# MarcVivas/gpu-physics-engine

Measured on AMD Instinct MI355X. Metric: physics_steps_per_sec, higher is better.
Workload: dtype f32+u32

## Files before the change

### gpu-physics-engine_amd/csrc/gpe_internal.h

```cpp
#pragma once

#include <hip/hip_runtime.h>
#include <stdint.h>

#include <string>
#include <vector>

#include "../../include/gpe.h"
#include "native_policy.h"

namespace gpe {

constexpr uint32_t kUnused = GPE_UNUSED_CELL_ID;
constexpr int kWave = 64;
constexpr int kStreamBlock = 256;
constexpr int kMaxStreamGrid = 256 * 8;

inline int stream_grid(uint64_t items, int per_block = kStreamBlock)
{
    uint64_t g = (items + per_block - 1) / per_block;
    if (g < 1) g = 1;
    if (g > (uint64_t)kMaxStreamGrid) g = kMaxStreamGrid;
    return (int)g;
}
// ... 243 lines not shown
constexpr int kNativeCtlSortsSeen = 38;
struct NativeState {
    NativePolicy policy;
    bool in_box = false;
    int32_t gx = 0, gy = 0;
    int passes = 4;
    uint32_t table_entries = 0;
    uint2 *block_table = nullptr;
    uint64_t table_cap = 0;
    uint32_t *keys = nullptr, *ids = nullptr;
    uint32_t *keys_b = nullptr, *ids_b = nullptr;
    uint64_t cap = 0;
    uint32_t *codes = nullptr;
    uint32_t *gkeys = nullptr, *gids = nullptr, *gkeys_b = nullptr, *gids_b = nullptr;
    uint64_t gcap = 0;
    uint2 *gtable = nullptr;
    uint32_t *ghist = nullptr;
    uint32_t ghist_set = 0;
    uint64_t gtable_cap = 0;
    const uint32_t *gsorted_ids_now = nullptr;
    uint32_t *exc_count = nullptr;
    uint2 *exc_entry = nullptr;
    uint64_t exc_tiles = 0, exc_cap = 0;
    uint4 *roster_hdr = nullptr;
    uint32_t *roster_ids = nullptr;
    uint64_t roster_cap = 0;
    TileBox tb;
    uint32_t *gho_count = nullptr;
    uint64_t gho_cap = 0;
    const uint32_t *gho_count_now = nullptr, *gho_entry_now = nullptr, *ghost_sort_now = nullptr;
    const uint32_t *exc_count_now = nullptr;
    const uint2 *exc_entry_now = nullptr;
    uint32_t *sorted_key = nullptr;
    bool sort_state_valid = false;
    uint64_t sorted_n = 0;
    uint32_t step_seq = 0;
    uint32_t collide_seq = 0;
    const uint32_t *fresh_word = nullptr;
    uint32_t reason = GPE_REASON_NO_PARTICLES;
    uint64_t native_steps = 0, compat_steps = 0;
    bool always_sort = false;
    int32_t blocks_x = 0, blocks_y = 0;
    int32_t bx0 = 0, by0 = 0;
    uint32_t *tile_ctl = nullptr;
    uint32_t *overflow1 = nullptr;
    uint64_t overflow_cap = 0;
    void *arena = nullptr;
    uint64_t arena_cap = 0;
    bool force = false;
    bool print_stats = false;
    uint32_t stat_calls = 0;
    uint32_t *host_stat = nullptr;
    uint32_t window_max = 0;
    unsigned long long *dbg_stamps = nullptr;
    uint4 *dbg_cycles = nullptr;
    uint64_t dbg_cycles_cap = 0;
};

constexpr int kShardMaxSlots = 9;
constexpr int kShardOwned = 0, kShardTotal = 1, kShardError = 2, kShardEpoch = 3, kShardHoles = 4;
constexpr int kShardSetWords = 8;
constexpr int kShardDoneTicket = 5;
struct ShardSlots {
    uint32_t n_slots;
    uint32_t rank[kShardMaxSlots];
    uint32_t send_off[kShardMaxSlots], send_cap_mig[kShardMaxSlots], send_cap_gho[kShardMaxSlots];
// ... 269 lines not shown
                            const uint32_t *ids, uint64_t n, float2 *pos_out, float2 *prev_out,
                            float *radius_out);
gpe_status launch_verlet(gpe_ctx *c, float2 *pos, float2 *prev, const float *radius, uint64_t n,
                         float dt);
gpe_status launch_build_cell_ids(gpe_ctx *c, const float2 *pos, const float *radius, uint64_t n,
                                 float cell_size, uint32_t *cell_ids, uint32_t *object_ids);
gpe_status sort_reserve(gpe_ctx *c, uint64_t n);
gpe_status sort_pairs(gpe_ctx *c, uint32_t *keys, uint32_t *vals, uint64_t n);
gpe_status sort_histogram(gpe_ctx *c, const uint32_t *keys, uint64_t n, uint32_t shift, uint32_t *hist256);
gpe_status sort_scatter_pass(gpe_ctx *c, const uint32_t *ka, const uint32_t *va, uint32_t *kb,
                             uint32_t *vb, uint64_t n, uint32_t shift);
gpe_status scan_reserve(gpe_ctx *c, uint64_t n);
gpe_status inclusive_scan(gpe_ctx *c, uint32_t *data, uint64_t n);
void sort_release(gpe_ctx *c);
void scan_release(gpe_ctx *c);
constexpr int kHistCopies = 8;
VerletParams verlet_params(const gpe_ctx *c, float dt);
gpe_status onesweep_reserve(gpe_ctx *c, uint64_t n);
void onesweep_release(gpe_ctx *c);
gpe_status onesweep_zero_hist(gpe_ctx *c);
struct OnesweepGate {
    const uint32_t *need = nullptr;
    uint32_t *key_copy = nullptr;
    uint32_t key_blocks_x = 1;
    uint64_t key_div_magic = 0;
    uint4 *table_reset = nullptr;
    uint64_t table_pairs = 0;
    uint32_t *fresh = nullptr;
    uint32_t *sorts = nullptr;
    uint32_t *sorts_seen = nullptr;
    int ticket_base = 0;
    const uint32_t *count_now = nullptr;
    uint32_t *sorted_count = nullptr;
};
gpe_status onesweep_sort(gpe_ctx *c, uint32_t *keys, uint32_t *vals, uint32_t *keys_b, uint32_t *vals_b,
                         uint64_t n, int passes, bool hist_ready, bool iota_vals, uint32_t **out_keys,
                         uint32_t **out_vals, bool bases_ready = false, uint2 *table = nullptr,
                         uint32_t table_entries = 0,
                         const uint32_t *hist_src = nullptr,
                         const OnesweepGate *gate = nullptr);
uint64_t remove_tiles(uint64_t n);
gpe_status launch_remove_count(gpe_ctx *c, const uint8_t *mask, float x, float y, float rr, uint32_t *tile_count,
                               unsigned long long *tile_key, unsigned long long *max_key);
gpe_status launch_remove_scatter(gpe_ctx *c, const uint8_t *mask, float x, float y, float rr,
                                 const uint32_t *tile_scanned, const uint32_t *uids = nullptr,
                                 uint32_t *uids_out = nullptr);
uint64_t query_tiles(uint64_t n);
gpe_status launch_query_count(gpe_ctx *c, bool box, const float *region, uint32_t *tile_count);
gpe_status launch_query_gather(gpe_ctx *c, bool box, const float *region, const uint32_t *tile_scanned,
                               uint32_t capacity, uint32_t *index_out, uint32_t *uid_out, float2 *pos_out,
                               float2 *prev_out, float *radius_out);
gpe_status launch_pick(gpe_ctx *c, float x, float y, unsigned long long *tile_key, unsigned long long *pick);
gpe_status native_configure(gpe_ctx *c);
bool native_should_run(gpe_ctx *c);
NativeStats native_read_stats(const NativeState &N);
void native_release(gpe_ctx *c);
gpe_status launch_shard_classify(gpe_ctx *c, const uint8_t *owner_of_block, const uint32_t *dest_mask_of_block,
                                 int32_t blocks_x, int32_t blocks_y, uint32_t my_rank, uint32_t *out_index,
                                 uint32_t *out_info, uint32_t *out_count, uint64_t out_capacity);
void shard_release(gpe_ctx *c);
void comm_release(gpe_ctx *c);
void ctl_release(gpe_ctx *c);
void shard_pack_args(gpe_ctx *c, PackArgs *P);
gpe_status coll_all_reduce_u32(gpe_ctx *c, uint32_t *d_buf, uint64_t count, uint32_t op);
gpe_status coll_all_to_all_u32(gpe_ctx *c, const uint32_t *d_send, const uint64_t *send_off, const uint64_t *send_cnt,
                               uint32_t *d_recv, const uint64_t *recv_off, const uint64_t *recv_cnt,
// ... 27 lines not shown
```

### gpu-physics-engine_amd/csrc/gpe_native.hip

```cpp
#include <assert.h>
#include <stdio.h>
#include <string.h>

#include <algorithm>
#include <string>
#include <utility>

#include "gpe_internal.h"
#include "native_launch.h"

namespace gpe {

template <class T>
static hipError_t release(gpe_ctx *c, T *&p)
{
    return dev_release(c, p);
}
template <class T>
static hipError_t reserve(gpe_ctx *c, T *&p, size_t payload, size_t slack, const char *tag)
{
    hipError_t e = release(c, p);
    if (e == hipSuccess) e = dev_reserve(c, &p, payload, slack, tag);
    return e;
}

void native_release(gpe_ctx *c)
{
    NativeState &N = c->native;
    void *bufs[] = {N.block_table, N.keys, N.ids, N.keys_b, N.ids_b, N.codes, N.sorted_key, N.gkeys, N.gids, N.gkeys_b,
                    N.gids_b, N.gtable, N.ghist, N.exc_count, N.gho_count, N.roster_hdr, N.roster_ids, N.tile_ctl,
                    N.overflow1, N.arena};
    for (void *b : bufs) (void)release(c, b);
    (void)release(c, N.dbg_stamps);
    (void)release(c, N.dbg_cycles);
    if (N.host_stat) (void)hipHostFree(N.host_stat);
    N = NativeState();
}

static gpe_status arena_reserve(gpe_ctx *c, uint64_t want);

NativeStats native_read_stats(const NativeState &N)
{
    assert(N.host_stat != nullptr);
    const auto word = [&](int k) { return __atomic_load_n(&N.host_stat[k], __ATOMIC_RELAXED); };
    NativeStats s;
    s.window_max = word(kStatWindowMax);
    s.arena = word(kStatArena);
    s.probe = word(kStatProbe);
    s.overflow = word(kStatOverflow);
    s.sub_tiles = word(kStatSubTiles);
    s.spills = word(kStatSpills);
    s.sorts = word(kStatSorts);
    s.overflow_new = word(kStatOverflowNew);
    s.halves_over = word(kStatHalvesOver);
    return s;
}

static void native_print_stats(gpe_ctx *c, const NativeStats &s)
{
    NativeState &N = c->native;
    if (N.print_stats && (++N.stat_calls & 127u) == 0)
        fprintf(stderr, "[gpe native] call %u: window max %u, arena slots used %u of %llu, 32x32 tiles over capacity %u, "
                        "quarters redone as 8x8 tiles %u, 8x8 tiles through the arena %u\n", N.stat_calls,
// ... 26 lines not shown
        for (int i = 0; i < 14; ++i) all += (double)h[i];
        for (int i = 0; i < 14; ++i)
            fprintf(stderr, "  P%d %.0f (%.1f%%)", i, h[16 + i] ? (double)h[i] / (double)h[16 + i] : 0.0, all > 0 ? 100.0 * (double)h[i] / all : 0.0);
        fprintf(stderr, "  (tiles %llu of %llu started)\n", h[16 + 6], h[16 + 0]);
        if (part == 1) (void)hipMemset(g_stamps, 0, 128 * 8);
    }
    return g_stamps;
}
#endif

static gpe_status native_prepare_step(gpe_ctx *c, uint32_t **sorted_ids, bool always_sort = false)
{
    NativeState &N = c->native;
    const uint64_t n = c->n;
    constexpr size_t kHistSet = (size_t)kHistCopies * 4 * 256;
    if (!c->os_ws.hist_clean) {
        GPE_HIP(c, hipMemsetAsync(c->os_ws.hist4, 0, 2 * kHistSet * sizeof(uint32_t), c->stream));
        c->os_ws.hist_clean = true;
        c->os_ws.hist_set = 0;
    }
    uint32_t *hist_now = c->os_ws.hist4 + (size_t)c->os_ws.hist_set * kHistSet;
    uint32_t *hist_next = c->os_ws.hist4 + (size_t)(c->os_ws.hist_set ^ 1u) * kHistSet;
    c->os_ws.hist_set ^= 1u;
    const uint32_t parity = (N.step_seq++) & 1u;
    const PreparePlan plan = N.policy.prepare(native_read_stats(N), always_sort, N.always_sort,
                                              (c->cfg.flags & GPE_FLAG_FUSED_HISTOGRAMS) != 0);
    const bool sharded = c->shard.on || c->use_order_keys || c->has_active_box;
    const bool kept_sharded = c->shard.on && c->shard.active && c->use_order_keys && N.gkeys != nullptr && !N.always_sort;
    const bool gated = N.passes >= 2 && (!sharded || kept_sharded);
    const bool reuse = gated && plan.keep_table && N.sort_state_valid && (kept_sharded || N.sorted_n == n) &&
                       N.exc_count != nullptr;
    const uint64_t pairs = ((uint64_t)N.table_entries + 1) / 2;
    const bool fuse_hist = plan.fuse_hist;
    HashGhosts hg;
    hg.sorted_count = N.tile_ctl + kCtlSortedCount;
    uint64_t g_bound = 0;
    if (kept_sharded) {
        const ShardState &SH = c->shard;
        g_bound = c->cap;
        const uint32_t epoch = __atomic_load_n(&SH.host_counts[kShardEpoch], __ATOMIC_ACQUIRE);
        if ((int32_t)(epoch - SH.begin_epoch) > 0) {
            const uint64_t gh = SH.host_counts[kShardTotal] >= SH.host_counts[kShardOwned]
                                    ? SH.host_counts[kShardTotal] - SH.host_counts[kShardOwned] : 0;
            g_bound = std::min<uint64_t>(c->cap, gh + std::max<uint64_t>(16384, gh / 4));
        }
        g_bound = std::min<uint64_t>(g_bound, n);
        hg.owned = SH.counts_now() + kShardOwned;
        hg.gkeys = N.gkeys; hg.gids = N.gids; hg.g_bound = g_bound;
        hg.gtable2 = (uint4 *)N.gtable; hg.gtable_pairs = pairs;
        hg.ghist_now = N.ghist + (size_t)N.ghist_set * kHistSet;
        hg.ghist_next = N.ghist + (size_t)(N.ghist_set ^ 1u) * kHistSet;
        N.ghist_set ^= 1u;
        hg.ghost_sort = N.tile_ctl + kCtlGhostSort + parity;
        hg.ghost_sort_next = N.tile_ctl + kCtlGhostSort + (parity ^ 1u);
        if (N.gho_count && N.gho_cap >= N.exc_tiles) {
            hg.gl_count = N.gho_count + (size_t)parity * N.exc_tiles;
            hg.gl_count_next = N.gho_count + (size_t)(parity ^ 1u) * N.exc_tiles;
            hg.gl_entry = N.gho_count + 2 * N.exc_tiles + (size_t)parity * N.exc_tiles * kGhostSlots;
        }
    }
    const uint64_t div_magic = ((1ull << 40) + (uint64_t)N.blocks_x - 1) / (uint64_t)N.blocks_x;
    {
        Scope s(c, "native/hash");
        const int grid = (int)std::min<uint64_t>(kHashGridMax, std::max<uint64_t>(1, n / (2ull * kHashBlock)));
        const uint32_t *n_valid = (c->shard.on && c->shard.active) ? c->shard.counts_now() + kShardTotal : nullptr;
        launch_native_hash(c, kept_sharded, grid, c->pos, c->radius, n, n_valid,
                           c->cell_size, N.gx, N.gy, N.bx0, N.by0, N.blocks_x, N.blocks_y, N.table_entries, N.keys,
                           N.codes, N.passes, hist_now, hist_next, c->os_ws.ctl, N.tile_ctl,
                           (uint4 *)N.block_table, gated ? 0ull : pairs,
                           N.host_stat, reuse ? N.sorted_key : nullptr, parity, div_magic,
                           N.exc_count ? N.exc_count + (size_t)parity * N.exc_tiles : nullptr,
                           N.exc_count ? N.exc_entry + (size_t)parity * N.exc_tiles * kExcSlots : nullptr,
                           N.exc_count ? N.exc_count + (size_t)(parity ^ 1u) * N.exc_tiles : nullptr, N.tb,
                           (uint32_t)std::max<uint64_t>(64, n >> 11),
                           fuse_hist ? 1u : 0u, hg);
        GPE_HIP(c, hipGetLastError());
    }
    uint32_t *sk = nullptr, *sv = nullptr;
    {
        Scope s(c, "native/sort");
        OnesweepGate g;
        g.need = N.tile_ctl + kCtlNeedSort + parity;
        if (reuse && !fuse_hist) {
            const int hgrid = (int)std::min<uint64_t>(kHistGatedGridMax, std::max<uint64_t>(1, n / (4ull * kHistGatedBlock)));
            launch_native_hist_gated(c, hgrid, N.keys, n, N.passes, hist_now, g.need);
            GPE_HIP(c, hipGetLastError());
        }
        g.fresh = N.tile_ctl + kCtlFresh + parity;
        g.sorts = N.tile_ctl + kCtlSorts;
        g.sorts_seen = N.tile_ctl + kCtlSortsSeen;
        if (gated) {
            g.key_copy = N.sorted_key; g.table_reset = (uint4 *)N.block_table; g.table_pairs = pairs;
            g.key_blocks_x = (uint32_t)N.blocks_x;
            g.key_div_magic = div_magic;
            g.count_now = hg.owned; g.sorted_count = N.tile_ctl + kCtlSortedCount;
        }
        GPE_TRY(onesweep_sort(c, N.keys, N.ids, N.keys_b, N.ids_b, n, N.passes, true, true, &sk, &sv, true,
                              N.block_table, N.table_entries, hist_now, &g));
    }
    (void)sk;
    N.gsorted_ids_now = nullptr;
    if (kept_sharded && g_bound > 0) {
        Scope s(c, "shard/ghost-sort");
        uint32_t *gk = nullptr, *gv = nullptr;
        OnesweepGate gg;
        gg.ticket_base = 8;
        gg.need = hg.ghost_sort;
        GPE_TRY(onesweep_sort(c, N.gkeys, N.gids, N.gkeys_b, N.gids_b, g_bound, N.passes, true, false, &gk, &gv, true,
                              N.gtable, N.table_entries, hg.ghist_now, &gg));
        (void)gk;
        N.gsorted_ids_now = gv;
    }
    N.sort_state_valid = gated;
    N.sorted_n = n;
    N.fresh_word = N.tile_ctl + kCtlFresh + parity;
    N.gho_count_now = hg.gl_count;
    N.gho_entry_now = hg.gl_entry;
    N.ghost_sort_now = hg.ghost_sort;
    N.exc_count_now = reuse ? N.exc_count + (size_t)parity * N.exc_tiles : nullptr;
    N.exc_entry_now = reuse ? N.exc_entry + (size_t)parity * N.exc_tiles * kExcSlots : nullptr;
    *sorted_ids = sv;
    return GPE_OK;
}
// ... 91 lines not shown
    if (!rosters_pay && N.roster_hdr) {
        N.roster_cap = 0;
        GPE_HIP(c, release(c, N.roster_hdr));
        GPE_HIP(c, release(c, N.roster_ids));
    }
    if (c->shard.on && c->has_active_box && N.gho_cap < N.exc_tiles) {
        N.gho_cap = 0;
        GPE_HIP(c, release(c, N.gho_count));
        if (reserve(c, N.gho_count, 2 * N.exc_tiles * (1 + (size_t)kGhostSlots) * sizeof(uint32_t), 64, "native.gho") == hipSuccess)
            N.gho_cap = N.exc_tiles;
    }
    if (N.gho_count) GPE_HIP(c, hipMemsetAsync(N.gho_count, 0, 2 * N.exc_tiles * sizeof(uint32_t), c->stream));
    if (rosters_pay && N.exc_count &&
        (c->cfg.flags & (GPE_FLAG_SORT_EVERY_STEP | GPE_FLAG_COUNTING_SORT_TILES)) == 0) {
        if (N.roster_cap < N.exc_tiles) {
            N.roster_cap = 0;
            GPE_HIP(c, release(c, N.roster_hdr));
            GPE_HIP(c, release(c, N.roster_ids));
            if (reserve(c, N.roster_hdr, N.exc_tiles * sizeof(uint4), 0, "native.roster_hdr") == hipSuccess &&
                reserve(c, N.roster_ids, N.exc_tiles * (size_t)kRosterCap * sizeof(uint32_t), 0, "native.roster_ids") == hipSuccess)
                N.roster_cap = N.exc_tiles;
            else { (void)release(c, N.roster_hdr); (void)release(c, N.roster_ids); }
        }
        if (N.roster_hdr) GPE_HIP(c, hipMemsetAsync(N.roster_hdr, 0, N.exc_tiles * sizeof(uint4), c->stream));
    }
    if (N.overflow_cap < tiles) {
        N.overflow_cap = 0;
        GPE_HIP(c, reserve(c, N.overflow1, (3 * tiles + 32 + 2 * kHintMax) * sizeof(uint32_t), 0, "native.overflow"));
        N.overflow_cap = tiles;
    }
    {
        const uint64_t want = std::min<uint64_t>(std::max<uint64_t>(c->cap, 1ull << 20), 32ull << 20);
        GPE_TRY(arena_reserve(c, std::max<uint64_t>(want, N.arena_cap)));
    }
    if (!N.tile_ctl) {
        GPE_HIP(c, reserve(c, N.tile_ctl, kCtlWords * sizeof(uint32_t), 0, "native.tile_ctl"));
        GPE_HIP(c, hipMemsetAsync(N.tile_ctl, 0, kCtlWords * sizeof(uint32_t), c->stream));
    }
    if (!N.host_stat) GPE_HIP(c, hipHostMalloc((void **)&N.host_stat, 64, hipHostMallocDefault));
    memset(N.host_stat, 0, 64);
    GPE_TRY(onesweep_reserve(c, c->cap));
    GPE_HIP(c, hipMemsetAsync(N.tile_ctl, 0, kCtlSorts * sizeof(uint32_t), c->stream));
    launch_native_check_box(c, c->pos, c->n,
                            (c->shard.on && c->shard.active) ? c->shard.counts_now() + kShardTotal : nullptr, c->cell_size, N.gx, N.gy,
                            N.tile_ctl + kCtlError);
    GPE_HIP(c, hipGetLastError());
    uint32_t flag = 1;
    GPE_HIP(c, hipMemcpyAsync(&flag, N.tile_ctl + kCtlError, sizeof(flag), hipMemcpyDeviceToHost, c->stream));
    GPE_HIP(c, hipStreamSynchronize(c->stream));
    GPE_HIP(c, hipMemsetAsync(N.tile_ctl, 0, kCtlSorts * sizeof(uint32_t), c->stream));
    N.reason = GPE_REASON_OUT_OF_BOX;
    if (flag != 0) return GPE_OK;
    N.in_box = true;
    const bool prof = c->profiling;
    c->profiling = false;
    uint32_t *ids = nullptr;
    gpe_status st = native_prepare_step(c, &ids, true);
    c->profiling = prof;
    GPE_TRY(st);
    launch_native_window_max(c, N.block_table, N.table_entries, N.blocks_x, N.blocks_y, N.tile_ctl + kCtlWindowMax);
    GPE_HIP(c, hipGetLastError());
    uint32_t wmax = 0xffffffffu;
    GPE_HIP(c, hipMemcpyAsync(&wmax, N.tile_ctl + kCtlWindowMax, sizeof(wmax), hipMemcpyDeviceToHost, c->stream));
    GPE_HIP(c, hipStreamSynchronize(c->stream));
    GPE_HIP(c, hipMemsetAsync(N.tile_ctl, 0, kCtlSorts * sizeof(uint32_t), c->stream));
    N.window_max = wmax;
// ... 236 lines not shown
```

### gpu-physics-engine_amd/csrc/k_native.hip

```cpp
#include <assert.h>
#include <stdio.h>
#include <stdlib.h>
#include <string.h>

#include <algorithm>
#include <type_traits>

#include "gpe_internal.h"
#include "k_pair.h"
#include "native_launch.h"

namespace gpe {

constexpr int kNatThreads = 512;
constexpr int kNatWaves = kNatThreads / 64;

__device__ __forceinline__ uint32_t nat_block_exclusive_scan(uint32_t v, uint32_t *s_w, uint32_t *total)
{
    const int lane = lane_id();
    const int w = (int)(threadIdx.x >> 6);
    const uint32_t inc = wave_inclusive_scan(v);
    if (lane == 63) s_w[w] = inc;
    __syncthreads();
    uint32_t base = 0, all = 0;
// ... 59 lines not shown
    }
    uint32_t over = 0;
    int k = 0;
#pragma unroll
    for (int y = -1; y <= 1; ++y) {
#pragma unroll
        for (int x = -1; x <= 1; ++x) {
            if (x == 0 && y == 0) continue;
            over |= (sx[x + 1] + sy[y + 1] < sq) ? (1u << k) : 0u;
            ++k;
        }
    }
    return over;
}

constexpr int kHashBatch = 2;
template <bool GHOSTS>
__global__ __launch_bounds__(kHashBlock, 8) void k_native_hash(const float2 *__restrict__ pos,
                                                            const float *__restrict__ radius, uint64_t n,
                                                            const uint32_t *__restrict__ n_valid_ptr,
                                                            float cell_size, int32_t gx, int32_t gy,
                                                            int32_t bx0, int32_t by0, int32_t blocks_x,
                                                            int32_t blocks_y, uint32_t pad_key,
                                                            uint32_t *__restrict__ keys,
                                                            uint32_t *__restrict__ codes, int digits,
                                                            uint32_t *hist4, uint32_t *__restrict__ hist_next,
                                                            uint32_t *__restrict__ os_ctl, uint32_t *tile_ctl,
                                                            uint4 *__restrict__ table2, uint64_t table_pairs,
                                                            uint32_t *__restrict__ host_stat,
                                                            const uint32_t *__restrict__ sorted_key, uint32_t parity,
                                                            uint64_t div_magic, uint32_t *__restrict__ exc_count,
                                                            uint2 *__restrict__ exc_entry,
                                                            uint32_t *__restrict__ exc_count_next, TileBox tb,
                                                            uint32_t straggler_limit, uint32_t fuse_always, HashGhosts G)
{
    (void)div_magic;
    __shared__ uint32_t s_hist[4 * 256];
    __shared__ uint32_t s_ghist[GHOSTS ? 4 * 256 : 1];
    __shared__ uint32_t s_sort_known;
    s_hist[threadIdx.x] = 0;
    if (GHOSTS) s_ghist[threadIdx.x] = 0;
    if (threadIdx.x == 0) s_sort_known = 0u;
    for (uint64_t i = (uint64_t)blockIdx.x * blockDim.x + threadIdx.x; i < table_pairs; i += (uint64_t)gridDim.x * blockDim.x)
        table2[i] = make_uint4(0xFFFFFFFFu, 0u, 0xFFFFFFFFu, 0u);
    if (GHOSTS)
    for (uint64_t i = (uint64_t)blockIdx.x * blockDim.x + threadIdx.x; i < G.gtable_pairs; i += (uint64_t)gridDim.x * blockDim.x)
        G.gtable2[i] = make_uint4(0xFFFFFFFFu, 0u, 0xFFFFFFFFu, 0u);
    if (exc_count_next) {
        const uint64_t nt = (uint64_t)tb.nx * (uint64_t)tb.ny;
        for (uint64_t i = (uint64_t)blockIdx.x * blockDim.x + threadIdx.x; i < nt; i += (uint64_t)gridDim.x * blockDim.x)
            exc_count_next[i] = 0;
    }
    if (GHOSTS && G.gl_count_next) {
        const uint64_t nt = (uint64_t)tb.nx * (uint64_t)tb.ny;
        for (uint64_t i = (uint64_t)blockIdx.x * blockDim.x + threadIdx.x; i < nt; i += (uint64_t)gridDim.x * blockDim.x)
            G.gl_count_next[i] = 0;
    }
    if (blockIdx.x == 0 && threadIdx.x < kCtlPerStepWords) {
        if (host_stat) {
            if (threadIdx.x == kCtlWindowMax) host_stat[kStatWindowMax] = tile_ctl[kCtlWindowMax];
            if (threadIdx.x == kCtlArena) host_stat[kStatArena] = tile_ctl[kCtlArena];
            if (threadIdx.x == kCtlOverflow1) {
                const uint32_t fresh_over = tile_ctl[kCtlOverflow1];
                host_stat[kStatOverflow] = fresh_over + tile_ctl[kCtlHintsSeen];
                host_stat[kStatOverflowNew] = fresh_over;
            }
            if (threadIdx.x == kCtlOverflow2) host_stat[kStatHalvesOver] = tile_ctl[kCtlOverflow2];
            if (threadIdx.x == kCtlSubTiles) host_stat[kStatSubTiles] = tile_ctl[kCtlSubTiles];
            if (threadIdx.x == kCtlSpills) host_stat[kStatSpills] = tile_ctl[kCtlSpills];
            if (threadIdx.x == 7) host_stat[kStatSorts] = tile_ctl[kCtlSorts];
        }
        tile_ctl[threadIdx.x] = 0;
    }
    if (blockIdx.x == 0) {
        for (int i = threadIdx.x; i < kHistCopies * 4 * 256; i += kHashBlock) hist_next[i] = 0;
        if (GHOSTS && G.ghist_next)
            for (int i = threadIdx.x; i < kHistCopies * 4 * 256; i += kHashBlock) G.ghist_next[i] = 0;
        if (threadIdx.x < 16) os_ctl[threadIdx.x] = 0;
        if (threadIdx.x == 0) {
            tile_ctl[kCtlNeedSort + (parity ^ 1u)] = 0;
            tile_ctl[kCtlFresh + (parity ^ 1u)] = 0;
            tile_ctl[parity ? kCtlStragglers0 : kCtlStragglers1] = 0;
            if (GHOSTS && G.ghost_sort_next) *G.ghost_sort_next = 0u;
            if (GHOSTS && G.gkeys && !G.gl_count) atomicOr(G.ghost_sort, 1u);
            if (!sorted_key) atomicOr(&tile_ctl[kCtlNeedSort + parity], 1u);
        }
    }
    __syncthreads();
    const uint64_t stride = (uint64_t)gridDim.x * blockDim.x;
    const uint64_t rounds = (n + stride - 1) / stride;
    uint64_t nv = n;
    if (n_valid_ptr) {
        nv = *n_valid_ptr;
        if (nv > n) { nv = n; if (threadIdx.x == 0) atomicOr(&tile_ctl[kCtlError], kErrBoundExceeded); }
    }
    uint64_t n_own = nv;
    if (GHOSTS && G.owned) n_own = min((uint64_t)*G.owned, nv);
    const uint64_t sorted_cnt = (sorted_key && G.sorted_count) ? (uint64_t)*G.sorted_count : ~0ull;
    if (GHOSTS && G.gkeys) {
        const uint64_t first = n - n_own;
        for (uint64_t j = first + (uint64_t)blockIdx.x * blockDim.x + threadIdx.x; j < G.g_bound; j += (uint64_t)gridDim.x * blockDim.x) {
            G.gkeys[j] = pad_key; G.gids[j] = 0u;
        }
        if (nv - n_own > G.g_bound && threadIdx.x == 0) atomicOr(&tile_ctl[kCtlError], kErrBoundExceeded);
    }
    bool oob = false, drifted = false;
    bool sort_known = sorted_key == nullptr;
    const bool fuse_hist = sorted_key == nullptr || fuse_always != 0u;
    for (uint64_t r0 = 0; r0 < rounds; r0 += kHashBatch) {
        float2 p[kHashBatch];
        float rad[kHashBatch];
        uint64_t idx[kHashBatch];
        uint32_t okey[kHashBatch];
#pragma unroll
        for (int u = 0; u < kHashBatch; ++u) {
            idx[u] = (r0 + u) * stride + (uint64_t)blockIdx.x * blockDim.x + threadIdx.x;
            const bool in = r0 + u < rounds && idx[u] < nv;
            p[u] = in ? pos[idx[u]] : make_float2(0.f, 0.f);
            rad[u] = in ? radius[idx[u]] : 0.f;
            okey[u] = (in && sorted_key) ? sorted_key[idx[u]] : 0u;
        }
#pragma unroll
        for (int u = 0; u < kHashBatch; ++u) {
            if (r0 + u >= rounds) break;
            const bool valid = idx[u] < n;
            uint32_t key = pad_key;
            if (valid && idx[u] >= nv) {
                keys[idx[u]] = pad_key; codes[idx[u]] = 0u;
                if (GHOSTS && G.gkeys && idx[u] - n_own < G.g_bound) { G.gkeys[idx[u] - n_own] = pad_key; G.gids[idx[u] - n_own] = 0u; }
            }
            const bool ghost = GHOSTS && idx[u] >= n_own;
            uint32_t gkey = 0;
            bool gvalid = false;
            if (idx[u] < nv) {
                const int32_t cx = cell_coord(p[u].x, cell_size), cy = cell_coord(p[u].y, cell_size);
                const int32_t lbx = (cx >> 3) - bx0, lby = (cy >> 3) - by0;
                const bool out = (cx < 0) | (cx >= gx) | (cy < 0) | (cy >= gy) | (lbx < 0) | (lbx >= blocks_x) |
                                 (lby < 0) | (lby >= blocks_y);
                oob |= out;
                key = out ? 0u : __umul24((uint32_t)lby, (uint32_t)blocks_x) + (uint32_t)lbx;
                if (GHOSTS && ghost && G.gkeys) {
// ... 15 lines not shown
                                (straggler ? kCodeStraggler : 0u);
                const uint64_t ms = ballot64(straggler);
                bool route = false;
                if (ms != 0 && !sort_known) {
                    sort_known = wave_lds_load(&s_sort_known) != 0u;
                    if (!sort_known) {
                        const int leader = (int)__builtin_ctzll(ms);
                        uint32_t before = 0;
                        if (lane_id() == leader)
                            before = atomicAdd(&tile_ctl[parity ? kCtlStragglers1 : kCtlStragglers0], (uint32_t)__popcll(ms));
                        before = (uint32_t)__builtin_amdgcn_readlane((int)before, leader);
                        if (before + (uint32_t)__popcll(ms) > straggler_limit) {
                            sort_known = true;
                            if (lane_id() == leader) { wave_lds_store(&s_sort_known, 1u); atomicOr(&tile_ctl[kCtlNeedSort + parity], 1u); }
                        } else route = true;
                    }
                }
                if (straggler && route) {
                    const int tx0 = max(tb.x0, (cx - (kConeRight + 1)) >> 5), tx1 = min(tb.x0 + tb.nx - 1, (cx + kConeLeft + 1) >> 5);
                    const int ty0 = max(tb.y0, (cy - (kConeUp + 1)) >> 5), ty1 = min(tb.y0 + tb.ny - 1, (cy + kConeDown + 1) >> 5);
                    for (int ty = ty0; ty <= ty1; ++ty)
                        for (int tx = tx0; tx <= tx1; ++tx) {
                            const uint32_t t = tb.index(tx, ty);
                            const uint32_t slot = atomicAdd(&exc_count[t], 1u);
                            if (slot < kExcSlots) exc_entry[(uint64_t)t * kExcSlots + slot] = make_uint2((uint32_t)idx[u], (uint32_t)cx | ((uint32_t)cy << 16));
                            else { drifted = true; atomicOr(&tile_ctl[kCtlNeedSort + parity], 1u); }
                        }
                }
            }
            if (fuse_hist) {
#pragma unroll
                for (int q = 0; q < 4; ++q)
                    if (q < digits) hist_add(s_hist + q * 256, (key >> (8 * q)) & 255u, valid);
            }
            if (GHOSTS && G.gkeys) {
#pragma unroll
                for (int q = 0; q < 4; ++q)
                    if (q < digits) hist_add(s_ghist + q * 256, (gkey >> (8 * q)) & 255u, gvalid);
            }
        }
    }
    if (GHOSTS && G.gl_count) {
        for (uint64_t i = n_own + (uint64_t)blockIdx.x * blockDim.x + threadIdx.x; i < nv; i += stride) {
            const float2 p = pos[i];
            const int32_t cx = cell_coord(p.x, cell_size), cy = cell_coord(p.y, cell_size);
            if ((cx < 0) | (cx >= gx) | (cy < 0) | (cy >= gy)) continue;
            const int tx0 = max(tb.x0, (cx - (kConeRight + 1)) >> 5), tx1 = min(tb.x0 + tb.nx - 1, (cx + kConeLeft + 1) >> 5);
            const int ty0 = max(tb.y0, (cy - (kConeUp + 1)) >> 5), ty1 = min(tb.y0 + tb.ny - 1, (cy + kConeDown + 1) >> 5);
            for (int ty = ty0; ty <= ty1; ++ty)
                for (int tx = tx0; tx <= tx1; ++tx) {
                    const uint32_t t = tb.index(tx, ty);
                    const uint32_t slot = atomicAdd(&G.gl_count[t], 1u);
                    if (slot < kGhostSlots) G.gl_entry[(uint64_t)t * kGhostSlots + slot] = (uint32_t)i;
                    else atomicOr(G.ghost_sort, 1u);
                }
        }
    }
    if (GHOSTS && G.gkeys && blockIdx.x == 0 && threadIdx.x < (uint32_t)digits) {
        const uint64_t ng = min(nv - n_own, G.g_bound);
        atomicAdd(&s_ghist[threadIdx.x * 256 + ((pad_key >> (8 * threadIdx.x)) & 255u)], (uint32_t)(G.g_bound - ng));
    }
    if (oob) atomicOr(&tile_ctl[kCtlError], kErrOutOfBox);
    if (ballot64(drifted) != 0 && lane_id() == 0) atomicOr(&tile_ctl[kCtlNeedSort + parity], 1u);
    __syncthreads();
    if ((threadIdx.x & 1u) == 0) {
        const uint32_t lo = s_hist[threadIdx.x], hi = s_hist[threadIdx.x + 1];
        if (fuse_hist && (lo | hi))
            __hip_atomic_fetch_add(
                reinterpret_cast<unsigned long long *>(&hist4[(blockIdx.x % kHistCopies) * 1024 + threadIdx.x]),
                (unsigned long long)lo | ((unsigned long long)hi << 32), __ATOMIC_RELAXED, __HIP_MEMORY_SCOPE_AGENT);
        if (GHOSTS && G.ghist_now) {
            const uint32_t glo = s_ghist[threadIdx.x], ghi = s_ghist[threadIdx.x + 1];
            if (glo | ghi)
                __hip_atomic_fetch_add(
                    reinterpret_cast<unsigned long long *>(&G.ghist_now[(blockIdx.x % kHistCopies) * 1024 + threadIdx.x]),
                    (unsigned long long)glo | ((unsigned long long)ghi << 32), __ATOMIC_RELAXED, __HIP_MEMORY_SCOPE_AGENT);
        }
    }
}

__global__ __launch_bounds__(kHistGatedBlock) void k_native_hist_gated(const uint32_t *__restrict__ keys, uint64_t n, int digits,
                                                                       uint32_t *__restrict__ hist4,
                                                                       const uint32_t *__restrict__ need)
{
    if (*need == 0u) return;
    __shared__ uint32_t s_hist[4 * 256];
    s_hist[threadIdx.x] = 0;
    __syncthreads();
    const uint64_t stride = (uint64_t)gridDim.x * blockDim.x;
    const uint64_t rounds = (n + stride - 1) / stride;
    for (uint64_t r = 0; r < rounds; ++r) {
        const uint64_t idx = r * stride + (uint64_t)blockIdx.x * blockDim.x + threadIdx.x;
        const bool valid = idx < n;
        const uint32_t key = valid ? keys[idx] : 0u;
#pragma unroll
        for (int q = 0; q < 4; ++q)
            if (q < digits) hist_add(s_hist + q * 256, (key >> (8 * q)) & 255u, valid);
// ... 2031 lines not shown
        A.tile_ctl[kCtlHintsSeen] = A.front_wgs != 0u ? used : 0u;
        A.tile_ctl[kCtlHints + A.hint_parity] = 0u;
    }
    if (work == 0) return;
    for (;;) {
        if (threadIdx.x == 0) s_item = atomicAdd(&A.tile_ctl[kCtlOverflowTicket], 1u);
        __syncthreads();
        const uint32_t i = s_item;
        __syncthreads();
        if (i >= work) break;
        uint32_t qx, qy;
        if (i >= work1) { const uint32_t h = A.overflow2[(i - work1) >> 1]; qx = (h & 0xFFFFu) * 2u + (i & 1u); qy = h >> 16; }
        else {
            const uint32_t parent = A.overflow1[i >> 2]; qx = (parent & 0xFFFFu) * 2u + (i & 1u); qy = (parent >> 16) * 2u + ((i >> 1) & 1u);
            if ((i & 3u) == 0u && threadIdx.x == 0) hint_tile(A, (int)(parent & 0xFFFFu), (int)(parent >> 16));
        }
#ifdef GPE_TILE_CYCLES
        const long long tq0 = clock64();
#endif
        resolve_quarter<ORD>(u, A, (int)qx, (int)qy);
#ifdef GPE_TILE_CYCLES
        if (g_tile_cycles && threadIdx.x == 0 && A.tb.holds((int)(qx >> 1), (int)(qy >> 1)))
            atomicAdd(&g_tile_cycles[A.tb.index((int)(qx >> 1), (int)(qy >> 1))].z, (uint32_t)(clock64() - tq0));
#endif
    }
}

void launch_native_hash(gpe_ctx *c, bool ghosts, int grid, const float2 *pos, const float *radius, uint64_t n,
                        const uint32_t *n_valid_ptr, float cell_size, int32_t gx, int32_t gy, int32_t bx0, int32_t by0,
                        int32_t blocks_x, int32_t blocks_y, uint32_t pad_key, uint32_t *keys, uint32_t *codes, int digits,
                        uint32_t *hist4, uint32_t *hist_next, uint32_t *os_ctl, uint32_t *tile_ctl, uint4 *table2,
                        uint64_t table_pairs, uint32_t *host_stat, const uint32_t *sorted_key, uint32_t parity,
                        uint64_t div_magic, uint32_t *exc_count, uint2 *exc_entry, uint32_t *exc_count_next, TileBox tb,
                        uint32_t straggler_limit, uint32_t fuse_always, const HashGhosts &G)
{
    const auto hash_kernel = ghosts ? k_native_hash<true> : k_native_hash<false>;
    hipLaunchKernelGGL(hash_kernel, dim3(grid), dim3(kHashBlock), 0, c->stream, pos, radius, n, n_valid_ptr, cell_size, gx,
                       gy, bx0, by0, blocks_x, blocks_y, pad_key, keys, codes, digits, hist4, hist_next, os_ctl, tile_ctl,
                       table2, table_pairs, host_stat, sorted_key, parity, div_magic, exc_count, exc_entry, exc_count_next,
                       tb, straggler_limit, fuse_always, G);
}

void launch_native_hist_gated(gpe_ctx *c, int grid, const uint32_t *keys, uint64_t n, int digits, uint32_t *hist4,
                              const uint32_t *need)
{
    hipLaunchKernelGGL(k_native_hist_gated, dim3(grid), dim3(kHistGatedBlock), 0, c->stream, keys, n, digits, hist4, need);
}

void launch_native_check_box(gpe_ctx *c, const float2 *pos, uint64_t n, const uint32_t *n_valid_ptr, float cell_size,
                             int32_t gx, int32_t gy, uint32_t *flag)
{
    hipLaunchKernelGGL(k_native_check_box, dim3(stream_grid(n)), dim3(kStreamBlock), 0, c->stream, pos, n, n_valid_ptr,
                       cell_size, gx, gy, flag);
}

void launch_native_window_max(gpe_ctx *c, const uint2 *table, uint32_t entries, int32_t blocks_x, int32_t blocks_y,
                              uint32_t *out_max)
{
    hipLaunchKernelGGL(k_native_window_max, dim3(stream_grid(entries)), dim3(kStreamBlock), 0, c->stream, table, entries,
                       blocks_x, blocks_y, out_max);
}

void launch_native_publish_probe(gpe_ctx *c, uint32_t *tile_ctl, uint32_t *host_stat)
{
    hipLaunchKernelGGL(k_native_publish_probe, dim3(1), dim3(64), 0, c->stream, tile_ctl, host_stat);
}

void launch_collide(gpe_ctx *c, CollideForm form, uint32_t grid, const CollideArgs &A)
{
    switch (form) {
    case CollideForm::DenseOrd:
        hipLaunchKernelGGL((k_collide_dense<kTileMain, kCapOrd, true>), dim3(grid), dim3(kNatThreads), 0, c->stream, A);
        break;
// ... 101 lines not shown
```

### gpu-physics-engine_amd/csrc/k_onesweep.hip

```cpp
#include <stdio.h>
#include <stdlib.h>

#include <algorithm>

#include "gpe_internal.h"

#ifdef GPE_OS_STAMPS
#define OS_STAMP(i)                                                                   \
    do {                                                                              \
        if (threadIdx.x == 0 && (s_tile & 63u) == 7u) {                               \
            const long long _t = clock64();                                           \
            atomicAdd(&ctl[16 + (i)], (uint32_t)(_t - _t_prev));                      \
            _t_prev = _t;                                                             \
        }                                                                             \
    } while (0)
#else
#define OS_STAMP(i) do {} while (0)
#endif

namespace gpe {

#ifndef GPE_OS_MINWAVES
#define GPE_OS_MINWAVES 4
#endif
// ... 117 lines not shown
    uint16_t slot[kOsItems];
#pragma unroll
    for (int k = 0; k < kOsItems; ++k) {
        const uint64_t idx = wave_base + (uint64_t)k * 64 + lane;
        const bool valid = idx < n;
        key[k] = valid ? keys_in[idx] : 0xffffffffu;
        if (IOTA) val[k] = (uint32_t)idx;
        else val[k] = valid ? vals_in[idx] : 0u;
    }
    if (G.key_copy) {
#pragma unroll
        for (int k = 0; k < kOsItems; ++k) {
            const uint64_t idx = wave_base + (uint64_t)k * 64 + lane;
            if (idx < n) {
                const uint32_t by = (uint32_t)(((uint64_t)key[k] * G.key_div_magic) >> 40);
                G.key_copy[idx] = (key[k] - by * G.key_blocks_x) | (by << 16);
            }
        }
        for (uint64_t i = (uint64_t)tile * kOsBlock + threadIdx.x; i < G.table_pairs; i += (uint64_t)gridDim.x * kOsBlock)
            G.table_reset[i] = make_uint4(0xFFFFFFFFu, 0u, 0xFFFFFFFFu, 0u);
        if (tile == 0 && threadIdx.x == 0) *G.sorted_count = G.count_now ? *G.count_now : (uint32_t)n;
    }
    if (G.fresh && tile == 0 && threadIdx.x == 0) {
        *G.fresh = 1u;
        const uint32_t before = atomicAdd(G.sorts, 1u);
        if (G.sorts_seen) *G.sorts_seen = before + 1u;
    }
    uint32_t digit_base = 0;
    if (hist_src) {
        uint32_t v = 0;
        if (threadIdx.x < 256) {
#pragma unroll
            for (int k = 0; k < kHistCopies; ++k) v += hist_src[k * 1024 + pass * 256 + threadIdx.x];
        }
        digit_base = os_block_exclusive_scan(v, s_w);
    }
#ifdef GPE_OS_STAMPS
    { uint32_t acc = 0; for (int k = 0; k < kOsItems; ++k) acc += key[k] + val[k]; asm volatile("" :: "v"(acc)); }
    OS_STAMP(0);
#endif
    uint32_t *wh = s_whist[w];
    u64 *wm = s_match[w];
    const u64 my_bit = 1ull << lane;
    constexpr int kBatch = 8;
    constexpr int kPeel = 4;
#pragma unroll
    for (int k0 = 0; k0 < kOsItems; k0 += kBatch) {
        u64 m[kBatch];
#pragma unroll
        for (int j = 0; j < kBatch; ++j) {
            const int k = k0 + j;
            const bool valid = wave_base + (uint64_t)k * 64 + lane < n;
            const uint32_t d = (key[k] >> shift) & 255u;
            u64 rem = ballot64(valid);
            u64 mine = 0ull;
#pragma unroll
            for (int it = 0; it < kPeel; ++it) {
                if (rem == 0) break;
                const int first = __builtin_amdgcn_readfirstlane((int)__builtin_ctzll(rem));
                const uint32_t d0 = (uint32_t)__builtin_amdgcn_readlane((int)d, first);
                const u64 same = ballot64(valid && d == d0) & rem;
                if (d == d0) mine = same;
                rem &= ~same;
            }
            const bool left = (rem >> lane) & 1ull;
            if (rem != 0) {
// ... 182 lines not shown
    if (passes < 1 || passes > 4) return fail(c, GPE_ERR_INVALID_ARG, "onesweep: passes must be 1..4");
    OnesweepWorkspace &ws = c->os_ws;
    const uint64_t tiles = os_tiles(n);
    if (!hist_ready) {
        Scope s(c, "sort/hist");
        GPE_TRY(onesweep_zero_hist(c));
        hipLaunchKernelGGL(k_os_hist4, dim3(stream_grid(n, kStreamBlock)), dim3(kStreamBlock), 0, c->stream, keys, n,
                           ws.hist_plain);
        GPE_HIP(c, hipGetLastError());
    }
    if (!(hist_ready && bases_ready)) {
        Scope s(c, "sort/prepare");
        hipLaunchKernelGGL(k_os_prepare, dim3(1), dim3(256), 0, c->stream, hist_ready ? ws.hist4 : ws.hist_plain, ws.bases4,
                           ws.ctl);
        GPE_HIP(c, hipGetLastError());
    }
    uint32_t *ka = keys, *va = vals, *kb = keys_b, *vb = vals_b;
    for (int p = 0; p < passes; ++p) {
        ws.epoch += 1;
        if (ws.epoch >= (1u << 30)) {
            GPE_HIP(c, hipMemsetAsync(ws.status, 0, ws.status_cap * sizeof(uint64_t), c->stream));
            ws.epoch = 1;
        }
        Scope s(c, "sort/onesweep");
        const bool iota = (p == 0 && iota_vals);
        const bool small = os_items(n) == kOsItemsSmall;
        const auto kern = small ? (iota ? k_os_pass<true, kOsItemsSmall> : k_os_pass<false, kOsItemsSmall>)
                                : (iota ? k_os_pass<true, kOsItems> : k_os_pass<false, kOsItems>);
        const bool last = p == passes - 1;
        OnesweepGate g;
        if (gate) {
            g.need = gate->need;
            g.ticket_base = gate->ticket_base;
            if (p == 0) {
                g.key_copy = gate->key_copy; g.table_reset = gate->table_reset; g.table_pairs = gate->table_pairs;
                g.key_blocks_x = gate->key_blocks_x; g.key_div_magic = gate->key_div_magic;
                g.count_now = gate->count_now; g.sorted_count = gate->sorted_count;
            }
            if (last) { g.fresh = gate->fresh; g.sorts = gate->sorts; g.sorts_seen = gate->sorts_seen; }
        }
        hipLaunchKernelGGL(kern, dim3((uint32_t)tiles), dim3(kOsBlock), 0, c->stream, ka, va, kb, vb, n,
                           (uint32_t)(8 * p), (uint32_t)p, ws.bases4, (u64 *)ws.status, ws.ctl, ws.epoch,
                           last ? table : nullptr, table_entries, (hist_ready && bases_ready) ? hist_src : nullptr, g);
        GPE_HIP(c, hipGetLastError());
        uint32_t *t = ka; ka = kb; kb = t;
        t = va; va = vb; vb = t;
    }
    if (out_keys) *out_keys = ka;
    if (out_vals) *out_vals = va;
#ifdef GPE_OS_STAMPS
    {
        static int calls = 0;
        if (++calls % 10 == 0) {
            uint32_t h[64];
            (void)hipStreamSynchronize(c->stream);
            (void)hipMemcpy(h, ws.ctl, sizeof(h), hipMemcpyDeviceToHost);
            const double nt = h[26] ? (double)h[26] : 1.0;
            fprintf(stderr, "[os stamps] n=%llu passes=%d sampled=%u  load %.0f  rank %.0f  reorder %.0f  lookback %.0f  write %.0f cyc;"
                            " hops/tile %.1f spins/tile %.1f\n", (unsigned long long)n, passes, h[26], h[16] / nt, h[17] / nt,
                    h[18] / nt, h[19] / nt, h[20] / nt, h[24] / nt, h[25] / nt);
        }
        (void)hipMemsetAsync(ws.ctl + 16, 0, 16 * sizeof(uint32_t), c->stream);
    }
#endif
    return GPE_OK;
}
// ... 3 lines not shown
```

### gpu-physics-engine_amd/csrc/native_launch.h

```cpp
#pragma once

#include "gpe_internal.h"

namespace gpe {

constexpr int kCtlOverflow1 = 0;
constexpr int kCtlOverflow2 = 1;
constexpr int kCtlHalfTicket = 7;
constexpr int kCtlWindowMax = 2;
constexpr int kCtlArena = 3;
constexpr int kCtlOverflowTicket = 4;
constexpr int kCtlSubTiles = 5;
constexpr int kCtlSpills = 6;
constexpr int kCtlPerStepWords = 8;
constexpr int kCtlHints = 11;
constexpr int kCtlHintsSeen = 13;
constexpr int kCtlError = 8;
constexpr int kCtlNeedSort = 34;
constexpr int kCtlFresh = 36;
constexpr int kCtlSorts = kNativeCtlSorts;
constexpr int kCtlStragglers0 = 9, kCtlStragglers1 = 15;
constexpr int kCtlSortedCount = 32;
constexpr int kCtlSortsSeen = kNativeCtlSortsSeen;
constexpr int kCtlGhostSort = 40;
constexpr int kCtlWords = 64;
constexpr uint32_t kExcSlots = 16;
constexpr uint32_t kGhostSlots = 256;
constexpr uint64_t kArenaBytesPerSlot = 37;
constexpr int kTileMain = 32;
struct HashGhosts {
    const uint32_t *owned = nullptr;
    uint32_t *gkeys = nullptr, *gids = nullptr;
    uint64_t g_bound = 0;
    uint4 *gtable2 = nullptr;
    uint64_t gtable_pairs = 0;
    const uint32_t *sorted_count = nullptr;
    uint32_t *ghist_now = nullptr, *ghist_next = nullptr;
    uint32_t *gl_count = nullptr, *gl_entry = nullptr, *gl_count_next = nullptr;
    uint32_t *ghost_sort = nullptr, *ghost_sort_next = nullptr;
};
constexpr int kHashBlock = 1024;
constexpr int kHashGridMax = 2048;
constexpr int kHistGatedBlock = 1024, kHistGatedGridMax = 2048;
#ifndef GPE_QMAX_MAIN_VALUE
#define GPE_QMAX_MAIN_VALUE 3
#endif
struct CollideArgs {
    const float2 *pos_in;
    const float *radius;
    float2 *pos_out;
    const uint32_t *sorted_ids;
    const uint32_t *codes;
    const uint2 *gtable;
    const uint32_t *gsorted_ids;
    const uint32_t *exc_count;
    const uint2 *exc_entry;
    TileBox tb;
    const uint32_t *gho_count;
    const uint32_t *gho_entry;
    const uint32_t *ghost_sort;
    const uint32_t *fresh;
    const uint2 *table;
    uint32_t entries;
    int32_t blocks_x, blocks_y;
    int32_t bx0, by0;
    const uint32_t *counts;
    float cell_size;
    float stiffness;
    int32_t gx, gy;
    int32_t tiles_x, tiles_y;
    uint32_t band_tiles;
    int32_t frame_l, frame_r, frame_b, frame_t;
    int32_t tile_x0, tile_y0;
    const uint32_t *order_keys;
    uint32_t *tile_ctl;
    uint32_t *overflow1;
    uint32_t overflow1_cap;
    uint32_t *overflow2;
    uint32_t quarters_of_halves;
    uint32_t *hints;
    uint32_t step_stamp, front_wgs, hint_parity;
    uint32_t hints_on;
    float *arena_px, *arena_py, *arena_rad;
    uint32_t *arena_id, *arena_hm, *arena_mem;
    uint8_t *arena_sblk;
    uint32_t arena_cap;
    float2 *prev;
    uint64_t n_owned;
    uint32_t fuse_verlet;
    VerletParams vp;
    uint4 *roster_hdr;
    uint32_t *roster_ids;
    const uint32_t *sorts_seen;
    uint32_t roster_write;
    unsigned long long *stamps;
    PackArgs pack;
};
constexpr int kRosterCap = GPE_QMAX_MAIN_VALUE * 512;

void launch_native_hash(gpe_ctx *c, bool ghosts, int grid, const float2 *pos, const float *radius, uint64_t n,
                        const uint32_t *n_valid_ptr, float cell_size, int32_t gx, int32_t gy, int32_t bx0, int32_t by0,
                        int32_t blocks_x, int32_t blocks_y, uint32_t pad_key, uint32_t *keys, uint32_t *codes, int digits,
                        uint32_t *hist4, uint32_t *hist_next, uint32_t *os_ctl, uint32_t *tile_ctl, uint4 *table2,
                        uint64_t table_pairs, uint32_t *host_stat, const uint32_t *sorted_key, uint32_t parity,
                        uint64_t div_magic, uint32_t *exc_count, uint2 *exc_entry, uint32_t *exc_count_next, TileBox tb,
                        uint32_t straggler_limit, uint32_t fuse_always, const HashGhosts &G);
void launch_native_hist_gated(gpe_ctx *c, int grid, const uint32_t *keys, uint64_t n, int digits, uint32_t *hist4,
                              const uint32_t *need);
void launch_native_check_box(gpe_ctx *c, const float2 *pos, uint64_t n, const uint32_t *n_valid_ptr, float cell_size,
                             int32_t gx, int32_t gy, uint32_t *flag);
void launch_native_window_max(gpe_ctx *c, const uint2 *table, uint32_t entries, int32_t blocks_x, int32_t blocks_y,
                              uint32_t *out_max);
void launch_native_publish_probe(gpe_ctx *c, uint32_t *tile_ctl, uint32_t *host_stat);
enum class CollideForm {
    Dense, DenseOrd,
    Direct, DirectFront, DirectOrd, DirectOrdFront,
    BorderOrd,
    Halves, HalvesOrd,
    Overflow, OverflowOrd,
};
void launch_collide(gpe_ctx *c, CollideForm form, uint32_t grid, const CollideArgs &A);
uint32_t dense_launch_band(uint32_t tiles_x, uint32_t tiles_y, bool eighths);
uint32_t dense_launch_grid(uint32_t tiles_x, uint32_t tiles_y, uint32_t band_tiles);

}
```

Baseline: 13390.

## Maintain radix histograms incrementally from key deltas instead of gated recount

When the sort table is reused and the run is not sharded, the hash kernel now adds only per-digit histogram deltas for particles whose cell key changed, rather than launching a separate gated histogram kernel over all keys. The onesweep sort adds a persistent kept histogram, stored in a double-buffered slot selected by a control word, to these deltas and writes the result back for the next step. This removes a full pass over the keys each step, at the cost of wave-level ballots and shared atomics in the hash kernel. It also adds cross-step state that must stay consistent with the actual sorted keys.

```diff
diff --git a/gpu-physics-engine_amd/csrc/gpe_internal.h b/gpu-physics-engine_amd/csrc/gpe_internal.h
--- a/gpu-physics-engine_amd/csrc/gpe_internal.h
+++ b/gpu-physics-engine_amd/csrc/gpe_internal.h
@@ -299,6 +299,7 @@
     const uint32_t *exc_count_now = nullptr;
     const uint2 *exc_entry_now = nullptr;
     uint32_t *sorted_key = nullptr;
+    uint32_t *kept_hist = nullptr;
     bool sort_state_valid = false;
     uint64_t sorted_n = 0;
     uint32_t step_seq = 0;
@@ -634,6 +635,9 @@
     int ticket_base = 0;
     const uint32_t *count_now = nullptr;
     uint32_t *sorted_count = nullptr;
+    uint32_t *kept = nullptr;
+    const uint32_t *kept_set = nullptr;
+    uint32_t kept_add = 0;
 };
 gpe_status onesweep_sort(gpe_ctx *c, uint32_t *keys, uint32_t *vals, uint32_t *keys_b, uint32_t *vals_b,
                          uint64_t n, int passes, bool hist_ready, bool iota_vals, uint32_t **out_keys,
diff --git a/gpu-physics-engine_amd/csrc/gpe_native.hip b/gpu-physics-engine_amd/csrc/gpe_native.hip
--- a/gpu-physics-engine_amd/csrc/gpe_native.hip
+++ b/gpu-physics-engine_amd/csrc/gpe_native.hip
@@ -28,7 +28,7 @@
 {
     NativeState &N = c->native;
     void *bufs[] = {N.block_table, N.keys, N.ids, N.keys_b, N.ids_b, N.codes, N.sorted_key, N.gkeys, N.gids, N.gkeys_b,
-                    N.gids_b, N.gtable, N.ghist, N.exc_count, N.gho_count, N.roster_hdr, N.roster_ids, N.tile_ctl,
+                    N.gids_b, N.gtable, N.ghist, N.kept_hist, N.exc_count, N.gho_count, N.roster_hdr, N.roster_ids, N.tile_ctl,
                     N.overflow1, N.arena};
     for (void *b : bufs) (void)release(c, b);
     (void)release(c, N.dbg_stamps);
@@ -121,6 +121,7 @@
                        N.exc_count != nullptr;
     const uint64_t pairs = ((uint64_t)N.table_entries + 1) / 2;
     const bool fuse_hist = plan.fuse_hist;
+    const bool delta_hist = reuse && !fuse_hist && !sharded && n <= kHistDeltaMaxN;
     HashGhosts hg;
     hg.sorted_count = N.tile_ctl + kCtlSortedCount;
     uint64_t g_bound = 0;
@@ -162,7 +163,7 @@
                            N.exc_count ? N.exc_entry + (size_t)parity * N.exc_tiles * kExcSlots : nullptr,
                            N.exc_count ? N.exc_count + (size_t)(parity ^ 1u) * N.exc_tiles : nullptr, N.tb,
                            (uint32_t)std::max<uint64_t>(64, n >> 11),
-                           fuse_hist ? 1u : 0u, hg);
+                           fuse_hist ? kHashHistFused : delta_hist ? kHashHistDelta : kHashHistGated, hg);
         GPE_HIP(c, hipGetLastError());
     }
     uint32_t *sk = nullptr, *sv = nullptr;
@@ -170,7 +171,7 @@
         Scope s(c, "native/sort");
         OnesweepGate g;
         g.need = N.tile_ctl + kCtlNeedSort + parity;
-        if (reuse && !fuse_hist) {
+        if (reuse && !fuse_hist && !delta_hist) {
             const int hgrid = (int)std::min<uint64_t>(kHistGatedGridMax, std::max<uint64_t>(1, n / (4ull * kHistGatedBlock)));
             launch_native_hist_gated(c, hgrid, N.keys, n, N.passes, hist_now, g.need);
             GPE_HIP(c, hipGetLastError());
@@ -178,6 +179,7 @@
         g.fresh = N.tile_ctl + kCtlFresh + parity;
         g.sorts = N.tile_ctl + kCtlSorts;
         g.sorts_seen = N.tile_ctl + kCtlSortsSeen;
+        g.kept = N.kept_hist; g.kept_set = N.tile_ctl + kCtlKeptSet; g.kept_add = delta_hist ? 1u : 0u;
         if (gated) {
             g.key_copy = N.sorted_key; g.table_reset = (uint4 *)N.block_table; g.table_pairs = pairs;
             g.key_blocks_x = (uint32_t)N.blocks_x;
@@ -335,6 +337,10 @@
     {
         const uint64_t want = std::min<uint64_t>(std::max<uint64_t>(c->cap, 1ull << 20), 32ull << 20);
         GPE_TRY(arena_reserve(c, std::max<uint64_t>(want, N.arena_cap)));
+    }
+    if (!N.kept_hist) {
+        GPE_HIP(c, reserve(c, N.kept_hist, 2 * 4 * 256 * sizeof(uint32_t), 0, "native.kept_hist"));
+        GPE_HIP(c, hipMemsetAsync(N.kept_hist, 0, 2 * 4 * 256 * sizeof(uint32_t), c->stream));
     }
     if (!N.tile_ctl) {
         GPE_HIP(c, reserve(c, N.tile_ctl, kCtlWords * sizeof(uint32_t), 0, "native.tile_ctl"));
diff --git a/gpu-physics-engine_amd/csrc/k_native.hip b/gpu-physics-engine_amd/csrc/k_native.hip
--- a/gpu-physics-engine_amd/csrc/k_native.hip
+++ b/gpu-physics-engine_amd/csrc/k_native.hip
@@ -115,7 +115,7 @@
                                                             uint64_t div_magic, uint32_t *__restrict__ exc_count,
                                                             uint2 *__restrict__ exc_entry,
                                                             uint32_t *__restrict__ exc_count_next, TileBox tb,
-                                                            uint32_t straggler_limit, uint32_t fuse_always, HashGhosts G)
+                                                            uint32_t straggler_limit, uint32_t hist_mode, HashGhosts G)
 {
     (void)div_magic;
     __shared__ uint32_t s_hist[4 * 256];
@@ -166,6 +166,7 @@
             tile_ctl[parity ? kCtlStragglers0 : kCtlStragglers1] = 0;
             if (GHOSTS && G.ghost_sort_next) *G.ghost_sort_next = 0u;
             if (GHOSTS && G.gkeys && !G.gl_count) atomicOr(G.ghost_sort, 1u);
+            tile_ctl[kCtlKeptSet] = tile_ctl[kCtlSorts] & 1u;
             if (!sorted_key) atomicOr(&tile_ctl[kCtlNeedSort + parity], 1u);
         }
     }
@@ -189,7 +190,8 @@
     }
     bool oob = false, drifted = false;
     bool sort_known = sorted_key == nullptr;
-    const bool fuse_hist = sorted_key == nullptr || fuse_always != 0u;
+    const bool fuse_hist = sorted_key == nullptr || hist_mode == kHashHistFused;
+    const bool delta_hist = !fuse_hist && hist_mode == kHashHistDelta;
     for (uint64_t r0 = 0; r0 < rounds; r0 += kHashBatch) {
         float2 p[kHashBatch];
         float rad[kHashBatch];
@@ -271,6 +273,19 @@
 #pragma unroll
                 for (int q = 0; q < 4; ++q)
                     if (q < digits) hist_add(s_hist + q * 256, (key >> (8 * q)) & 255u, valid);
+            } else if (delta_hist) {
+                const uint32_t old = __umul24(okey[u] >> 16, (uint32_t)blocks_x) + (okey[u] & 0xFFFFu);
+                const bool moved = valid && key != old;
+                if (ballot64(moved) != 0) {
+#pragma unroll
+                    for (int q = 0; q < 4; ++q) {
+                        const uint32_t d_new = (key >> (8 * q)) & 255u, d_old = (old >> (8 * q)) & 255u;
+                        if (q < digits && moved && d_new != d_old) {
+                            atomicAdd(&s_hist[q * 256 + d_new], 1u);
+                            atomicAdd(&s_hist[q * 256 + d_old], 0xFFFFFFFFu);
+                        }
+                    }
+                }
             }
             if (GHOSTS && G.gkeys) {
 #pragma unroll
@@ -302,6 +317,12 @@
     if (oob) atomicOr(&tile_ctl[kCtlError], kErrOutOfBox);
     if (ballot64(drifted) != 0 && lane_id() == 0) atomicOr(&tile_ctl[kCtlNeedSort + parity], 1u);
     __syncthreads();
+    if (delta_hist) {
+        const uint32_t v = s_hist[threadIdx.x];
+        if (v)
+            __hip_atomic_fetch_add(&hist4[(blockIdx.x % kHistCopies) * 1024 + threadIdx.x], v, __ATOMIC_RELAXED,
+                                   __HIP_MEMORY_SCOPE_AGENT);
+    }
     if ((threadIdx.x & 1u) == 0) {
         const uint32_t lo = s_hist[threadIdx.x], hi = s_hist[threadIdx.x + 1];
         if (fuse_hist && (lo | hi))
@@ -2399,13 +2420,13 @@
                         uint32_t *hist4, uint32_t *hist_next, uint32_t *os_ctl, uint32_t *tile_ctl, uint4 *table2,
                         uint64_t table_pairs, uint32_t *host_stat, const uint32_t *sorted_key, uint32_t parity,
                         uint64_t div_magic, uint32_t *exc_count, uint2 *exc_entry, uint32_t *exc_count_next, TileBox tb,
-                        uint32_t straggler_limit, uint32_t fuse_always, const HashGhosts &G)
+                        uint32_t straggler_limit, uint32_t hist_mode, const HashGhosts &G)
 {
     const auto hash_kernel = ghosts ? k_native_hash<true> : k_native_hash<false>;
     hipLaunchKernelGGL(hash_kernel, dim3(grid), dim3(kHashBlock), 0, c->stream, pos, radius, n, n_valid_ptr, cell_size, gx,
                        gy, bx0, by0, blocks_x, blocks_y, pad_key, keys, codes, digits, hist4, hist_next, os_ctl, tile_ctl,
                        table2, table_pairs, host_stat, sorted_key, parity, div_magic, exc_count, exc_entry, exc_count_next,
-                       tb, straggler_limit, fuse_always, G);
+                       tb, straggler_limit, hist_mode, G);
 }
 
 void launch_native_hist_gated(gpe_ctx *c, int grid, const uint32_t *keys, uint64_t n, int digits, uint32_t *hist4,
diff --git a/gpu-physics-engine_amd/csrc/k_onesweep.hip b/gpu-physics-engine_amd/csrc/k_onesweep.hip
--- a/gpu-physics-engine_amd/csrc/k_onesweep.hip
+++ b/gpu-physics-engine_amd/csrc/k_onesweep.hip
@@ -173,6 +173,11 @@
         if (threadIdx.x < 256) {
 #pragma unroll
             for (int k = 0; k < kHistCopies; ++k) v += hist_src[k * 1024 + pass * 256 + threadIdx.x];
+            if (G.kept) {
+                const uint32_t set = *G.kept_set & 1u;
+                if (G.kept_add) v += G.kept[set * 1024 + pass * 256 + threadIdx.x];
+                if (tile == 0) G.kept[(set ^ 1u) * 1024 + pass * 256 + threadIdx.x] = v;
+            }
         }
         digit_base = os_block_exclusive_scan(v, s_w);
     }
@@ -421,6 +426,7 @@
         if (gate) {
             g.need = gate->need;
             g.ticket_base = gate->ticket_base;
+            g.kept = gate->kept; g.kept_set = gate->kept_set; g.kept_add = gate->kept_add;
             if (p == 0) {
                 g.key_copy = gate->key_copy; g.table_reset = gate->table_reset; g.table_pairs = gate->table_pairs;
                 g.key_blocks_x = gate->key_blocks_x; g.key_div_magic = gate->key_div_magic;
diff --git a/gpu-physics-engine_amd/csrc/native_launch.h b/gpu-physics-engine_amd/csrc/native_launch.h
--- a/gpu-physics-engine_amd/csrc/native_launch.h
+++ b/gpu-physics-engine_amd/csrc/native_launch.h
@@ -23,6 +23,7 @@
 constexpr int kCtlSortedCount = 32;
 constexpr int kCtlSortsSeen = kNativeCtlSortsSeen;
 constexpr int kCtlGhostSort = 40;
+constexpr int kCtlKeptSet = 42;
 constexpr int kCtlWords = 64;
 constexpr uint32_t kExcSlots = 16;
 constexpr uint32_t kGhostSlots = 256;
@@ -39,6 +40,10 @@
     uint32_t *gl_count = nullptr, *gl_entry = nullptr, *gl_count_next = nullptr;
     uint32_t *ghost_sort = nullptr, *ghost_sort_next = nullptr;
 };
+constexpr uint32_t kHashHistGated = 0;
+constexpr uint32_t kHashHistFused = 1;
+constexpr uint32_t kHashHistDelta = 2;
+constexpr uint64_t kHistDeltaMaxN = 4ull << 20;
 constexpr int kHashBlock = 1024;
 constexpr int kHashGridMax = 2048;
 constexpr int kHistGatedBlock = 1024, kHistGatedGridMax = 2048;
@@ -104,7 +109,7 @@
                         uint32_t *hist4, uint32_t *hist_next, uint32_t *os_ctl, uint32_t *tile_ctl, uint4 *table2,
                         uint64_t table_pairs, uint32_t *host_stat, const uint32_t *sorted_key, uint32_t parity,
                         uint64_t div_magic, uint32_t *exc_count, uint2 *exc_entry, uint32_t *exc_count_next, TileBox tb,
-                        uint32_t straggler_limit, uint32_t fuse_always, const HashGhosts &G);
+                        uint32_t straggler_limit, uint32_t hist_mode, const HashGhosts &G);
 void launch_native_hist_gated(gpe_ctx *c, int grid, const uint32_t *keys, uint64_t n, int digits, uint32_t *hist4,
                               const uint32_t *need);
 void launch_native_check_box(gpe_ctx *c, const float2 *pos, uint64_t n, const uint32_t *n_valid_ptr, float cell_size,
```

Measured after the change: 13610, median of 6. 1.02x the previous value.
